# mit-acl/rl_collision_avoidance

Measured on AMD Instinct MI355X. Metric: agent-steps/sec (env.step) at 4 agents x 8192 worlds per GPU, higher is better.
Workload: dtype f64

## Files before the change

### include/cavoid.h

```cpp
#ifndef CAVOID_H
#define CAVOID_H
#include <stdint.h>

#ifdef __cplusplus
extern "C" {
#endif

#define CAVOID_ABI_VERSION 3
#define CAVOID_MAX_ACTIONS 32
#define CAVOID_MAX_AGENTS 64

#define CAVOID_F_AT_GOAL 0x01u
#define CAVOID_F_RAN_OUT 0x02u
#define CAVOID_F_IN_COLL 0x04u
#define CAVOID_F_WAS_AT_GOAL 0x08u
#define CAVOID_F_WAS_IN_COLL 0x10u
#define CAVOID_F_PRESENT 0x20u
#define CAVOID_F_LEARNING 0x40u
#define CAVOID_F_POLICY_SHIFT 8
#define CAVOID_F_POLICY_MASK 7u
enum { CAVOID_POLICY_EXTERNAL = 0, CAVOID_POLICY_STATIC = 1, CAVOID_POLICY_NONCOOP = 2, CAVOID_POLICY_RVO = 3, CAVOID_POLICY_FROZEN_NET = 4 };
#define CAVOID_F_DONE_MASK 0x07u

enum { CAVOID_SORT_CLOSEST_LAST = 0, CAVOID_SORT_CLOSEST_FIRST = 1, CAVOID_SORT_TIME_TO_IMPACT = 2 };
// ... 91 lines not shown
int cavoid_step_autoreset_n(cavoid_env *env, const int32_t *actions, int64_t action_stride, int32_t n_steps, int64_t out_step_stride,
                            float *obs, float *rewards, uint8_t *done, uint8_t *game_over, void *stream);

enum {
    CAVOID_FORM_NONE = 0,
    CAVOID_FORM_STEP = 1,
    CAVOID_FORM_QUAD = 2,
    CAVOID_FORM_RVO = 3,
    CAVOID_FORM_LOOP_PF = 4,
    CAVOID_FORM_LOOP = 5,
    CAVOID_FORM_PIPE = 6,
    CAVOID_FORM_RELAY = 7,
    CAVOID_FORM_CROWD = 8
};
int32_t cavoid_last_step_form(const cavoid_env *env, int32_t *relay_consumers);

int cavoid_step_continuous_autoreset(cavoid_env *env, const float *actions , float *obs, float *rewards, uint8_t *done,
                                     uint8_t *game_over, void *stream);
int cavoid_step_continuous_autoreset_n(cavoid_env *env, const float *actions, int64_t action_stride, int32_t n_steps, int64_t out_step_stride,
                                       float *obs, float *rewards, uint8_t *done, uint8_t *game_over, void *stream);

int32_t cavoid_packed_width(const cavoid_env *env);
int cavoid_reset_packed(cavoid_env *env, const uint8_t *world_mask, float *packed, void *stream);
int cavoid_observe_packed(cavoid_env *env, float *packed, void *stream);
int cavoid_step_packed(cavoid_env *env, const int32_t *actions, float *packed, uint8_t *game_over, void *stream);
int cavoid_step_autoreset_packed(cavoid_env *env, const int32_t *actions, int64_t action_stride, int32_t n_steps, int64_t out_step_stride,
                                 float *packed, uint8_t *game_over, void *stream);
int cavoid_step_continuous_autoreset_packed(cavoid_env *env, const float *actions, int64_t action_stride, int32_t n_steps,
                                            int64_t out_step_stride, float *packed, uint8_t *game_over, void *stream);

// ... 124 lines not shown
```

### rl_collision_avoidance_amd/_lib.py

```python
from __future__ import annotations

import ctypes as C
import os

from .build import LIB_PATH as _DEFAULT_LIB_PATH

LIB_PATH = os.environ.get("CAVOID_LIB", _DEFAULT_LIB_PATH)

MAX_ACTIONS = 32
MAX_AGENTS = 64
TILE_MAX_AGENTS = 16
ABI_VERSION = 3

F_AT_GOAL, F_RAN_OUT, F_IN_COLL, F_WAS_AT_GOAL, F_WAS_IN_COLL, F_PRESENT, F_LEARNING = 1, 2, 4, 8, 16, 32, 64
F_POLICY_SHIFT = 8
F_POLICY_MASK = 7
POLICY_EXTERNAL, POLICY_STATIC, POLICY_NONCOOP, POLICY_RVO, POLICY_FROZEN_NET = 0, 1, 2, 3, 4
F_DONE_MASK = 7
COMM_FORCE_RCCL = 1
STEP_FORMS = ("NONE", "STEP", "QUAD", "RVO", "LOOP_PF", "LOOP", "PIPE", "RELAY", "CROWD")


class CavoidCfg(C.Structure):
    _fields_ = [
# ... 53 lines not shown
        self.code = code


_P = C.c_void_p
SYMBOLS = [
    ("cavoid_abi_version", C.c_int, []),
    ("cavoid_strerror", C.c_char_p, [C.c_int]),
    ("cavoid_last_hip_error", C.c_int, []),
    ("cavoid_default_cfg", C.c_int, [C.POINTER(CavoidCfg), C.c_int32, C.c_int32]),
    ("cavoid_default_actions", C.c_int, [_P, C.POINTER(C.c_int32)]),
    ("cavoid_create", C.c_int, [C.POINTER(CavoidCfg), C.c_int64, C.c_int64, C.c_int, C.POINTER(_P)]),
    ("cavoid_destroy", None, [_P]),
    ("cavoid_num_worlds", C.c_int64, [_P]),
    ("cavoid_obs_width", C.c_int32, [_P]),
    ("cavoid_last_step_form", C.c_int32, [_P, C.POINTER(C.c_int32)]),
    ("cavoid_seed", C.c_int, [_P, C.c_uint64, _P, _P]),
    ("cavoid_get_episode", C.c_int, [_P, _P, _P]),
    ("cavoid_pool_refresh", C.c_int, [_P, C.c_uint32, _P]),
    ("cavoid_set_state", C.c_int, [_P, _P, _P, _P, _P]),
    ("cavoid_get_state", C.c_int, [_P, _P, _P, _P, _P]),
    ("cavoid_reset", C.c_int, [_P, _P, _P, _P]),
    ("cavoid_observe", C.c_int, [_P, _P, _P]),
    ("cavoid_step", C.c_int, [_P, _P, _P, _P, _P, _P, _P]),
    ("cavoid_step_continuous", C.c_int, [_P, _P, _P, _P, _P, _P, _P]),
    ("cavoid_step_autoreset", C.c_int, [_P, _P, _P, _P, _P, _P, _P]),
    ("cavoid_step_autoreset_n", C.c_int, [_P, _P, C.c_int64, C.c_int32, C.c_int64, _P, _P, _P, _P, _P]),
    ("cavoid_step_continuous_autoreset", C.c_int, [_P, _P, _P, _P, _P, _P, _P]),
    ("cavoid_step_continuous_autoreset_n", C.c_int, [_P, _P, C.c_int64, C.c_int32, C.c_int64, _P, _P, _P, _P, _P]),
    ("cavoid_step_continuous_autoreset_packed", C.c_int, [_P, _P, C.c_int64, C.c_int32, C.c_int64, _P, _P, _P]),
    ("cavoid_step_autoreset_n_timed", C.c_int, [_P, _P, C.c_int64, C.c_int32, C.c_int32, C.c_int64, _P, _P, _P, _P, _P, C.POINTER(C.c_float)]),
# ... 73 lines not shown
```

### rl_collision_avoidance_amd/batched_env.py

```python
from __future__ import annotations

import ctypes as C
from typing import Optional, Tuple

import numpy as np
import torch

from . import _lib
from .config import EnvConfig

_SORT = {"closest_last": 0, "closest_first": 1, "time_to_impact": 2}
_DYN = {"unicycle": 0, "unicycle_max_turn_rate": 1, "holonomic": 2}


def make_cfg(config: Optional[EnvConfig] = None, **overrides) -> _lib.CavoidCfg:
    config = config or EnvConfig()
    cfg = _lib.CavoidCfg()
    N = int(config.MAX_NUM_AGENTS_IN_ENVIRONMENT)
    M = int(config.MAX_NUM_OTHER_AGENTS_OBSERVED)
    _lib.check(_lib.lib().cavoid_default_cfg(C.byref(cfg), N, M), "cavoid_default_cfg")
    cfg.dt = config.DT
    cfg.near_goal_threshold = config.NEAR_GOAL_THRESHOLD
    cfg.max_time_ratio = config.MAX_TIME_RATIO
    cfg.collision_dist = config.COLLISION_DIST
# ... 181 lines not shown
    def refresh_pool(self, epoch: int) -> None:
        _lib.check(self._lib.cavoid_pool_refresh(self._h, int(epoch) & 0xFFFFFFFF, self._stream()), "cavoid_pool_refresh")

    @property
    def episode(self) -> torch.Tensor:
        out = torch.empty((self.num_worlds,), dtype=torch.int32, device=self.device)
        _lib.check(self._lib.cavoid_get_episode(self._h, self._ptr(out), self._stream()), "cavoid_get_episode")
        return out

    @property
    def last_step_form(self) -> Tuple[str, int]:
        nc = C.c_int32(0)
        form = self._lib.cavoid_last_step_form(self._h, C.byref(nc))
        return _lib.STEP_FORMS[form], int(nc.value)

    def set_state(self, state_f64: torch.Tensor, state_f32: torch.Tensor, flags: torch.Tensor) -> None:
        A = self.num_worlds * self.max_agents
        f64 = self._want(state_f64, (4, A), torch.float64, "state_f64")
        f32 = self._want(state_f32, (5, A), torch.float32, "state_f32")
        fl = self._want(flags, (A,), torch.int32, "flags")
        _lib.check(self._lib.cavoid_set_state(self._h, self._ptr(f64), self._ptr(f32), self._ptr(fl), self._stream()),
                   "cavoid_set_state")

    def get_state(self) -> Tuple[torch.Tensor, torch.Tensor, torch.Tensor]:
        A = self.num_worlds * self.max_agents
        f64 = torch.empty((4, A), dtype=torch.float64, device=self.device)
        f32 = torch.empty((5, A), dtype=torch.float32, device=self.device)
        fl = torch.empty((A,), dtype=torch.int32, device=self.device)
        _lib.check(self._lib.cavoid_get_state(self._h, self._ptr(f64), self._ptr(f32), self._ptr(fl), self._stream()),
                   "cavoid_get_state")
# ... 164 lines not shown
```

### rl_collision_avoidance_amd/csrc/cavoid_capi.hip

```cpp
#include <hip/hip_runtime.h>
#include <hip/hip_ext.h>

#include <cmath>
#include <cstdlib>
#include <cstring>
#include <new>

#include "cavoid.h"
#include "cavoid_host.hpp"
#include "cavoid_kernels.hpp"
#include "cavoid_launch.hpp"
#include "cavoid_crowd.hpp"

using namespace cavoid;

thread_local int g_last_hip_error = 0;

extern "C" int cavoid_abi_version(void) { return CAVOID_ABI_VERSION; }

extern "C" int cavoid_last_hip_error(void) { return g_last_hip_error; }

extern "C" const char *cavoid_strerror(int code) {
    switch (code) {
        case CAVOID_OK: return "ok";
// ... 333 lines not shown
    if (capturing) e->ahead_always = true;
    if (!e->ahead_always && e->ahead_primed && e->ahead_budget >= n_steps + 1) return CAVOID_OK;
    const int64_t waves = (e->W + e->k.wpw - 1) / e->k.wpw;
    const bool in_place = e->ahead_always;
    const dim3 grid((unsigned)((waves + 3) / 4), in_place ? 1u : (e->ahead_primed ? 4u : 32u)), block(256);
    const uint32_t *hi_in = e->ahead_hi[e->ahead_cur];
    uint32_t *hi_out = e->ahead_hi[in_place ? e->ahead_cur : (e->ahead_cur ^ 1)];
    hipEvent_t ev_fill = (timed_start && !capturing) ? *timed_start : nullptr;
    if (ev_fill) *timed_start = nullptr;
    const int rc = dispatch_n(e->cfg.max_agents, EnvNs{}, [&](auto n) -> int {
        launch_kernel(ahead_fill_kernel<decltype(n)::value>, grid, block, 0, s, ev_fill, nullptr, e->k, e->st.episode, hi_in, hi_out, e->pool, e->ahead_R);
        return CAVOID_OK;
    });
    if (rc != CAVOID_OK) return rc;
    HIP_TRY(hipGetLastError());
    if (!in_place) e->ahead_cur ^= 1;
    if (!capturing) { e->ahead_primed = true; e->ahead_budget = e->ahead_R; }
    return CAVOID_OK;
}
void cavoid_ahead_consumed(cavoid_env *e, int32_t n_steps) {
    if (!e || e->ahead_R <= 0) return;
    e->ahead_budget = e->ahead_budget > n_steps ? e->ahead_budget - n_steps : 0;
}

static int fill_pool(cavoid_env *e, hipStream_t s) {
    if (e->ahead_R > 0) {
        e->ahead_budget = 0;
        e->ahead_primed = false;
        HIP_TRY(hipMemsetAsync(e->ahead_hi[0], 0xFF, 2 * (size_t)e->W * sizeof(uint32_t), s));
        return CAVOID_OK;
    }
    if (e->pool_size <= 0) return CAVOID_OK;
    HIP_TRY(hipMemsetAsync(e->pool_episode, 0xFF, (size_t)e->pool_size * sizeof(uint32_t), s));
    KCfg k = e->k;
    k.num_worlds = e->pool_size;
    k.world_offset = 0;
    k.pool_size = 0;
    KState st{};
// ... 118 lines not shown
    return launch<MODE_STEP>(e, io, static_cast<hipStream_t>(stream));
}

static int launch_autoreset(cavoid_env *e, KIO io, const int32_t *actions, int64_t action_stride, int32_t n_steps, int64_t out_step_stride,
                            hipStream_t s, hipEvent_t ev_start = nullptr, hipEvent_t ev_stop = nullptr, const float *cont = nullptr) {
    if (e->cfg.dynamics == CAVOID_DYN_HOLONOMIC && !cont) return CAVOID_EINVAL;
    if (n_steps < 1 || action_stride < 0) return CAVOID_EINVAL;
    if (cont && n_steps > 1 && action_stride != 0 && action_stride < 2 * e->A) return CAVOID_EINVAL;
    if (out_step_stride != 0 && out_step_stride < e->W) return CAVOID_EINVAL;
    io.out_step_stride = n_steps > 1 ? out_step_stride : 0;
    io.actions = actions;
    io.cont = cont;
    io.action_stride = action_stride;
    io.n_steps = n_steps;
    e->last_form = CAVOID_FORM_NONE;
    if (int rc = cavoid_ahead_prepare(e, n_steps, s, &ev_start)) return rc;
    const int rc = (n_steps > 1 || e->prefetch_single)
                       ? cavoid_launch_multistep(e, io, e->latency_mode != 0, s, ev_start, ev_stop)
                       : launch<MODE_STEP_AUTORESET>(e, io, s, ev_start, ev_stop);
    cavoid_ahead_consumed(e, n_steps);
    return rc;
}

extern "C" int cavoid_step_autoreset(cavoid_env *e, const int32_t *actions, float *obs, float *rew, uint8_t *done, uint8_t *game_over, void *stream) {
    if (step_args(e, actions, rew, done, game_over) != CAVOID_OK) return CAVOID_EINVAL;
    return launch_autoreset(e, plain_io(e, obs, rew, done, game_over), actions, 0, 1, 0, static_cast<hipStream_t>(stream));
}

extern "C" int cavoid_step_autoreset_n(cavoid_env *e, const int32_t *actions, int64_t action_stride, int32_t n_steps, int64_t out_step_stride,
                                       float *obs, float *rew, uint8_t *done, uint8_t *game_over, void *stream) {
    if (step_args(e, actions, rew, done, game_over) != CAVOID_OK || n_steps < 0) return CAVOID_EINVAL;
    if (n_steps == 0) return CAVOID_OK;
    return launch_autoreset(e, plain_io(e, obs, rew, done, game_over), actions, action_stride, n_steps, out_step_stride,
                            static_cast<hipStream_t>(stream));
}
// ... 118 lines not shown
```

### rl_collision_avoidance_amd/csrc/cavoid_kernels.hpp

```cpp
#pragma once
#include <hip/hip_runtime.h>
#include <stdint.h>

#include "cavoid.h"

namespace cavoid {

#ifdef CAVOID_TRACE
__device__ unsigned long long *g_trace = nullptr;
#define CAVOID_STAMP(k)                                                                \
    do {                                                                               \
        if (lane == 0 && g_trace) g_trace[wave * 16 + (k)] = (unsigned long long)clock64(); \
    } while (0)
#else
#define CAVOID_STAMP(k) do { } while (0)
#endif

#define CAVOID_RARE(x) __builtin_expect(!!(x), 0)
#ifndef CAVOID_SKIP
#define CAVOID_SKIP 0
#endif

constexpr double kPi = 3.14159265358979323846;
constexpr int kTileMaxAgents = 16;
// ... 767 lines not shown
    a.gx = r.gx; a.gy = r.gy; a.radius = r.radius; a.pref = r.pref;
    a.flags = r.flags;
    a.vx = a.vy = 0.0;
    a.speed = 0.0f;
}

template <int N>
__device__ __forceinline__ void new_episode(const KCfg &c, const PoolRec *pool, uint32_t gw, uint32_t ep, int i, Agent &a) {
    if (c.pool_size > 0) {
        load_pool(pool, (int64_t)pool_index(c, gw, ep) * N + i, a);
    } else {
        generate_agent<N>(c, gw, ep, i, a);
    }
}

template <int N>
__device__ __forceinline__ void ahead_fill_wave(const KCfg &c, const uint32_t *episode, const uint32_t *hi_in, uint32_t *hi_out, PoolRec *ahead, const int need,
                                                const int64_t wave, const int lane, const int y, const int ny, double *sc_d, float *sc_r) {
    const int wpw = c.wpw, lanes_used = wpw * N;
    const int lw = lane / N, i = lane - lw * N;
    const int64_t w = wave * wpw + lw;
    const bool active = lane < lanes_used && w < c.num_worlds;
    const int base = lane < lanes_used ? lw * N : 0;
    uint32_t ep = 0u, fh = 0u;
    if (active) {
        ep = episode[w];
        fh = hi_in[w];
        if (fh == 0xFFFFFFFFu || (int32_t)(fh - ep) < 0) fh = ep;
    }
    const uint32_t target = ep + (uint32_t)need;
    int missing = active ? (int)(int32_t)(target - fh) : 0;
    missing = missing < 0 ? 0 : missing;
    int trips = missing;
#pragma unroll
    for (int o = 32; o > 0; o >>= 1) { const int v = __shfl_xor(trips, o, 64); trips = v > trips ? v : trips; }
    const uint32_t gw = (uint32_t)(c.world_offset + w);
    for (int k = y; k < trips; k += ny) {
        const uint32_t e = fh + 1u + (uint32_t)k;
        const bool fresh = active && k < missing;
        Agent a;
        absent_agent(a);
        if (c.gen_mode == 1) generate_world_v2<N>(c, gw, e, i, base, lane, fresh, sc_d, sc_d + 64, sc_d + 128, sc_d + 192, sc_r, a);
        else if (fresh) generate_agent<N>(c, gw, e, i, a);
        if (fresh) {
            PoolRec r;
            r.px = a.px; r.py = a.py; r.heading = a.heading; r.t_rem = a.t_rem;
            r.gx = a.gx; r.gy = a.gy; r.radius = a.radius; r.pref = a.pref;
            r.flags = a.flags; r.pad[0] = r.pad[1] = r.pad[2] = 0u;
            ahead[((int64_t)w * c.ahead + (int64_t)(e & (uint32_t)(c.ahead - 1))) * N + i] = r;
        }
    }
    if (active && i == 0 && y == 0) hi_out[w] = missing > 0 ? target : fh;
}

template <int N>
__global__ void __launch_bounds__(256) ahead_fill_kernel(const KCfg c, const uint32_t *episode, const uint32_t *hi_in, uint32_t *hi_out, PoolRec *ahead, const int need) {
    __shared__ double sh_d[4][4 * 64];
    __shared__ float sh_r[4][64];
    const int wave_in_block = threadIdx.x >> 6;
    ahead_fill_wave<N>(c, episode, hi_in, hi_out, ahead, need, (int64_t)blockIdx.x * 4 + wave_in_block, threadIdx.x & 63, (int)blockIdx.y, (int)gridDim.y,
                       sh_d[wave_in_block], sh_r[wave_in_block]);
}

constexpr double kRvoEps = 1e-5;
__device__ __forceinline__ double det2(double ax, double ay, double bx, double by) { return ax * by - ay * bx; }

struct Line { double px, py, dx, dy; };
// ... 731 lines not shown
```

### rl_collision_avoidance_amd/csrc/cavoid_launch.hpp

```cpp
#pragma once
#include <hip/hip_runtime.h>
#include <hip/hip_ext.h>

#include <type_traits>

#include "cavoid.h"
#include "cavoid_host.hpp"
#include "cavoid_kernels.hpp"

struct cavoid_env {
    int device = 0;
    int64_t W = 0, A = 0, world_offset = 0;
    cavoid_cfg cfg{};
    cavoid::KCfg k{};
    cavoid::KState st{};
    cavoid::PoolRec *pool = nullptr;
    uint32_t *pool_episode = nullptr;
    int64_t pool_size = 0;
    int ahead_R = 0;
    uint32_t *ahead_hi[2] = {nullptr, nullptr};
    int ahead_cur = 0;
    int ahead_budget = 0;
    bool ahead_primed = false;
    bool ahead_always = false;
    void *slab = nullptr;
    void *pool_slab = nullptr;
    double *d_actions = nullptr;
    int waves_per_block = 4;
    int grid = 0;
    int pipeline = 2;
    int relay_consumers = 3;
    int latency_mode = 0;
    int quad = -1;
    int prefetch_single = 0;
    int last_form = CAVOID_FORM_NONE;
    int last_relay_consumers = 0;
    hipEvent_t ev0 = nullptr, ev1 = nullptr;
};

// ... 28 lines not shown

template <class K, class... Args>
static inline void launch_kernel(K kernel, dim3 grid, dim3 block, size_t lds, hipStream_t s, hipEvent_t ev_start, hipEvent_t ev_stop,
                                 const Args &...args) {
    if (ev_start || ev_stop) hipExtLaunchKernelGGL(kernel, grid, block, lds, s, ev_start, ev_stop, 0, args...);
    else hipLaunchKernelGGL(kernel, grid, block, lds, s, args...);
}

#ifdef CAVOID_TRACE
static inline int set_trace(unsigned long long *dev_ptr) {
    HIP_TRY(hipMemcpyToSymbol(HIP_SYMBOL(g_trace), &dev_ptr, sizeof(dev_ptr)));
    return CAVOID_OK;
}
#endif

static inline int note_form(cavoid_env *e, int rc, int form, int relay_consumers = 0) {
    if (rc == CAVOID_OK) {
        e->last_form = form;
        e->last_relay_consumers = relay_consumers;
    }
    return rc;
}

template <int MODE, bool RVO = false>
static inline int launch_on(cavoid_env *e, const KCfg &k, const KState &st, int grid_x, const KIO &io, hipStream_t s,
                     hipEvent_t ev_start, hipEvent_t ev_stop) {
    const dim3 grid(grid_x), block(64 * e->waves_per_block);
    const int row = io.obs ? io.obs_stride : k.width;
    int tile = (k.tile_rows * row + 3) & ~3;
    if (tile < k.park_floats) tile = k.park_floats;
// ... 24 lines not shown
        constexpr int N = decltype(n)::value;
        const size_t lds = pipe_lds_fixed_bytes<N>() + tail;
        if (lds > 65536) return CAVOID_EUNSUPPORTED;
        launch_kernel(env_pipe_kernel<N, RVO>, grid, block, lds, s, ev_start, ev_stop, k, e->st, e->pool, io);
        return CAVOID_OK;
    });
    if (rc != CAVOID_OK) return rc;
    HIP_TRY(hipGetLastError());
    return CAVOID_OK;
}

}

int cavoid_ahead_prepare(cavoid_env *e, int32_t n_steps, hipStream_t s, hipEvent_t *timed_start = nullptr);
void cavoid_ahead_consumed(cavoid_env *e, int32_t n_steps);
int cavoid_launch_relay(cavoid_env *e, const cavoid::KIO &io, hipStream_t s, hipEvent_t ev_start, hipEvent_t ev_stop);
int cavoid_launch_quad(cavoid_env *e, const cavoid::KIO &io, hipStream_t s, hipEvent_t ev_start, hipEvent_t ev_stop);
int cavoid_launch_multistep(cavoid_env *e, const cavoid::KIO &io, bool prefetch, hipStream_t s, hipEvent_t ev_start, hipEvent_t ev_stop);
int cavoid_launch_rvo(cavoid_env *e, int mode, const cavoid::KIO &io, hipStream_t s, hipEvent_t ev_start, hipEvent_t ev_stop);
int cavoid_launch_crowd(cavoid_env *e, int mode, const cavoid::KCfg &k, const cavoid::KState &st, int64_t worlds, const cavoid::KIO &io,
                        hipStream_t s, hipEvent_t ev_start, hipEvent_t ev_stop);
#ifdef CAVOID_TRACE
int cavoid_debug_trace_multistep(unsigned long long *dev_ptr);
int cavoid_debug_trace_rvo(unsigned long long *dev_ptr);
int cavoid_debug_trace_relay(unsigned long long *dev_ptr);
int cavoid_debug_trace_quad(unsigned long long *dev_ptr);
#endif
```

### rl_collision_avoidance_amd/csrc/cavoid_relay.hip

```cpp
#include "cavoid_launch.hpp"
#include "cavoid_relay.hpp"

using namespace cavoid;

template <int N>
static int relay_allow_lds() {
    static bool allowed = false;
    if (!allowed) {
        HIP_TRY(hipFuncSetAttribute(reinterpret_cast<const void *>(env_relay_kernel<N>), hipFuncAttributeMaxDynamicSharedMemorySize, (int)kRelayLdsLimit));
        allowed = true;
    }
    return CAVOID_OK;
}

int cavoid_launch_relay(cavoid_env *e, const KIO &io, hipStream_t s, hipEvent_t ev_start, hipEvent_t ev_stop) {
    const KCfg &k = e->k;
    if (k.rvo_enabled || k.pool_size <= 0 || !io.obs || !io.actions || io.cont) return CAVOID_EUNSUPPORTED;
    if (k.switches & kSwSkipDonePairs) return CAVOID_EUNSUPPORTED;
    const int64_t tiles = (e->W + k.wpw - 1) / k.wpw;
    if (tiles > 512) return CAVOID_EUNSUPPORTED;
    if (e->cfg.max_agents > kRelayMaxAgents) return CAVOID_EUNSUPPORTED;
    const int row = io.obs_stride;
    const int tile_floats = (k.tile_rows * row + 3) & ~3;
    if (k.tile_rows < k.wpw * e->cfg.max_agents) return CAVOID_EUNSUPPORTED;
    const dim3 grid((unsigned)tiles);
    int used_nc = 0;
    const int rc = dispatch_n(e->cfg.max_agents, RelayNs{}, [&](auto n) -> int {
        constexpr int N = decltype(n)::value;
        int nc = e->relay_consumers;
        while (nc > 1 && relay_lds_fixed_bytes<N>() + (size_t)nc * tile_floats * sizeof(float) > kRelayLdsLimit) --nc;
        const size_t lds = relay_lds_fixed_bytes<N>() + (size_t)nc * tile_floats * sizeof(float);
        if (lds > kRelayLdsLimit || (nc < 2 && e->relay_consumers >= 2)) return CAVOID_EUNSUPPORTED;
        if (lds > 65536) {
            const int rc_opt = relay_allow_lds<N>();
            if (rc_opt != CAVOID_OK) return rc_opt;
        }
        used_nc = nc;
        launch_kernel(env_relay_kernel<N>, grid, dim3(64 * (3 + nc)), lds, s, ev_start, ev_stop, k, e->st, e->pool, io);
        return CAVOID_OK;
    });
    if (rc != CAVOID_OK) return rc;
    HIP_TRY(hipGetLastError());
    return note_form(e, CAVOID_OK, CAVOID_FORM_RELAY, used_nc);
}

#ifdef CAVOID_TRACE
int cavoid_debug_trace_relay(unsigned long long *dev_ptr) { return set_trace(dev_ptr); }
#endif
```

### rl_collision_avoidance_amd/csrc/cavoid_relay.hpp

```cpp
#pragma once
#include "cavoid_kernels.hpp"

namespace cavoid {

constexpr int kRelayMaxAgents = 6;
template <int N>
__host__ __device__ constexpr int relay_ring() { return N <= 5 ? 8 : 4; }
constexpr size_t kRelayLdsLimit = 80 * 1024;
constexpr int kRelayActRing = 64;
constexpr int kRelayActAhead = 48;
constexpr int kRelayEvq = 8;

struct RelaySeq {
    int spec;
    int stage;
    int res;
    int fin;
    int act;
    int ev;
    int nxt;
    int cons[kRelayMaxConsumers];
    int cfin[kRelayMaxConsumers];
    int coop[2];
    int kernarg[2];
// ... 8 lines not shown
#endif
#ifndef CAVOID_RELAY_PRIO_D
#define CAVOID_RELAY_PRIO_D 3
#endif
#ifndef CAVOID_RELAY_PRIO_P
#define CAVOID_RELAY_PRIO_P 3
#endif
#ifndef CAVOID_RELAY_PRIO_L
#define CAVOID_RELAY_PRIO_L 0
#endif
#ifndef CAVOID_RELAY_PRIO_C
#define CAVOID_RELAY_PRIO_C 1
#endif
#ifndef CAVOID_RELAY_ABL
#define CAVOID_RELAY_ABL 0
#endif
__device__ __forceinline__ int relay_role_of(int wv, int NC) {
    if (NC == 3) return (int)(((unsigned)CAVOID_RELAY_ORDER >> (4 * wv)) & 15u);
    return wv;
}
constexpr int kRelayCoopWaves = 3;
constexpr int kRelayCoopFromN = 4;
template <int N>
struct RelayCoop {
    static constexpr int K = Others<N>::K;
    uint64_t key[K][64];
    uint32_t bits[K][64];
};
template <int N>
__host__ __device__ constexpr size_t relay_coop_bytes() { return N >= kRelayCoopFromN ? sizeof(RelayCoop<N>) : 0; }
// ... 204 lines not shown
        neighbour_features(e, (float)e.prll_x, (float)e.prll_y, rx, ry, q, feat[o]);
    }
}

struct RelayArgs { KCfg c; KState s; const PoolRec *pool; KIO io; };
template <class T>
__device__ __forceinline__ void relay_load_args(T &dst, const __attribute__((address_space(4))) T *src) {
    static_assert(sizeof(T) % 4 == 0, "whole words");
    const __attribute__((address_space(4))) uint32_t *w = (const __attribute__((address_space(4))) uint32_t *)src;
    uint32_t d[sizeof(T) / 4];
#pragma unroll
    for (int k = 0; k < (int)(sizeof(T) / 4); ++k) d[k] = w[k];
    __builtin_memcpy(&dst, d, sizeof(T));
}
template <int N>
__device__ __forceinline__ void relay_coop_last(unsigned char *smem) {
    unsigned char *sp = smem + lds_floats_block() * sizeof(float);
    RelaySeq *seq = reinterpret_cast<RelaySeq *>(sp); sp += sizeof(RelaySeq) + kRelayEvq * sizeof(unsigned long long);
    const unsigned long long kp = (unsigned long long)(uint32_t)relay_peek(&seq->kernarg[0]) | ((unsigned long long)(uint32_t)relay_peek(&seq->kernarg[1]) << 32);
    typedef const __attribute__((address_space(4))) RelayArgs *ArgP;
    const ArgP ka = (ArgP)kp;
    KCfg c;
    KIO io;
    relay_load_args(c, &ka->c);
    relay_load_args(io, &ka->io);
    RelayTent *tents = reinterpret_cast<RelayTent *>(sp); sp += relay_ring<N>() * sizeof(RelayTent) + sizeof(RelayNxt);
    RelayRes *ress = reinterpret_cast<RelayRes *>(sp); sp += relay_ring<N>() * sizeof(RelayRes) + kRelayActRing * 64;
    RelayCoop<N> *coopb = reinterpret_cast<RelayCoop<N> *>(sp); sp += relay_coop_bytes<N>();
    float *tiles = reinterpret_cast<float *>(sp);
    const int lane0 = threadIdx.x & 63;
// ... 39 lines not shown
        gapf[o] = 0.0f;
#pragma unroll
        for (int q = 0; q < kFeat; ++q) feat[o][q] = 0.0f;
    }
    if (c.switches != 0u) relay_pair_part<N, true>(c, ao, e, present, as, pw, lane0, co, gapf, feat);
    else relay_pair_part<N, false>(c, ao, e, present, as, pw, lane0, co, gapf, feat);
    relay_coop_arrive(&seq->coop[0], lane0);
    Key key[K];
    uint32_t valid = 0u;
    if (N == 1) key[0].set(kKeySentinel, 0u);
#pragma unroll
    for (int o = 0; o < N - 1; ++o) {
        key[o].v = co.key[o][lane0];
        valid |= (co.bits[o][lane0] & 2u) ? (1u << o) : 0u;
    }
    if (t - NC >= 0) relay_wait_bounded(&seq->cons[cid_l], t - NC + 1);
    const int rows_active = (int)worlds_here * N;
    assemble_obs<N, false, true, ArrayStage<N>, NoHook, false, PartOthers>(c, ao, e, active, lane0, as, key, gapf, feat, valid, tile, nullptr,
                                                                           rows_active, ostride, false, 0.0f, 0.0f, wave, NoHook(), false, nullptr,
                                                                           PartOthers{pw, kRelayCoopWaves});
    if (pw == 0 && active && lane0 < rows_active) {
        const int M = c.max_other;
        const int m = __popc(valid);
        const int first = m > M ? m - M : 0;
        const int kept = m - first;
        write_row_head(tile + lane0 * ostride, ao, e, present, kept, kept, M, packed, c.width, rew_c, done_c);
    }
    relay_coop_arrive(&seq->coop[1], lane0);
    if (io.out_step_stride == 0)
        for (int o = 0; o < NC; ++o) relay_wait_bounded(&seq->cfin[o], 1);
// ... 3 lines not shown
        const bool lines = ((rows_active * ostride) & 31) == 0 && (reinterpret_cast<uintptr_t>(dst) & 127) == 0;
        if (io.out_step_stride != 0 && lines) flush_tile<4, true, true>(tile, dst, rows_active * ostride, pw * 64 + lane0, 64 * kRelayCoopWaves);
        else if (io.out_step_stride != 0) flush_tile<4, true>(tile, dst, rows_active * ostride, pw * 64 + lane0, 64 * kRelayCoopWaves);
        else flush_tile<4>(tile, dst, rows_active * ostride, pw * 64 + lane0, 64 * kRelayCoopWaves);
    }
    if (pw == 0 && active) {
        if (!packed) {
            io.rew[slot_w * N + a_idx0] = rew_c;
            io.done[slot_w * N + a_idx0] = (ctl_c & 1u) ? 1 : 0;
        }
        if (i0 == 0) io.game_over[slot_w + w] = (ctl_c & 2u) ? 1 : 0;
    }
    if (pw == 0) RELAY_MARK(29);
}

template <int N>
__global__ void __launch_bounds__(64 * (3 + kRelayMaxConsumers), 1) env_relay_kernel(const KCfg c, const KState s, const PoolRec *pool, const KIO io) {
    extern __shared__ __attribute__((aligned(16))) unsigned char smem[];
    unsigned char *sp = smem;
    double *lds_tab = reinterpret_cast<double *>(sp); sp += lds_floats_block() * sizeof(float);
    RelaySeq *seq = reinterpret_cast<RelaySeq *>(sp); sp += sizeof(RelaySeq);
    unsigned long long *evq = reinterpret_cast<unsigned long long *>(sp); sp += kRelayEvq * sizeof(unsigned long long);
    RelayTent *tents = reinterpret_cast<RelayTent *>(sp); sp += relay_ring<N>() * sizeof(RelayTent);
    RelayNxt *nbuf = reinterpret_cast<RelayNxt *>(sp); sp += sizeof(RelayNxt);
    RelayRes *ress = reinterpret_cast<RelayRes *>(sp); sp += relay_ring<N>() * sizeof(RelayRes);
    unsigned char *actring = sp; sp += kRelayActRing * 64;
    RelayCoop<N> *coopb = reinterpret_cast<RelayCoop<N> *>(sp); sp += relay_coop_bytes<N>();
    float *tiles = reinterpret_cast<float *>(sp);

    const int NC = (blockDim.x >> 6) - 3;
    const int role = relay_role_of(threadIdx.x >> 6, NC);
    const int lane0 = threadIdx.x & 63;
// ... 4 lines not shown
    const int64_t w0 = wave * wpw;
    const int lw = lane0 / N, i0 = lane0 - lw * N;
    const int64_t w = w0 + lw;
    const bool active = lane0 < lanes_used && w < c.num_worlds;
    const int base0 = lane0 < lanes_used ? lw * N : 0;
    const int64_t a_idx0 = w * N + i0;
    const bool packed = io.packed != 0;
    int64_t worlds_here = c.num_worlds - w0;
    if (worlds_here > wpw) worlds_here = wpw;
    if (worlds_here < 0) worlds_here = 0;
    const int n_steps = io.n_steps;
    constexpr bool kCoop = N >= kRelayCoopFromN;
    const bool coop_role = role < 2 || role == 2 + NC;

    if (role == 0 && lane0 < (int)(sizeof(RelaySeq) / sizeof(int))) reinterpret_cast<int *>(seq)[lane0] = 0;
    if constexpr (kCoop) {
        if (role == 0 && lane0 == 0) {
            const unsigned long long kp = (unsigned long long)__builtin_amdgcn_kernarg_segment_ptr();
            seq->kernarg[0] = (int)(uint32_t)kp; seq->kernarg[1] = (int)(uint32_t)(kp >> 32);
            seq->tile_id = (int)blockIdx.x;
        }
    }

    if (role == 0) {
        __builtin_amdgcn_s_setprio(CAVOID_RELAY_PRIO_D);
        RELAY_MARK(20);
        KCfg cd = c;
        asm volatile("" : "+s"(cd.dt), "+s"(cd.near_goal_sq), "+s"(cd.actions_fp32), "+s"(cd.dynamics),
                     "+s"(cd.timeout_enabled), "+s"(cd.switches));
        const RelayTrig trig = relay_trig_constants();
        Agent a;
        a.px = a.py = a.heading = a.t_rem = a.vx = a.vy = 0.0;
        a.gx = a.gy = a.radius = a.pref = a.speed = 0.0f;
        a.flags = 0u;
        uint32_t episode = 0u;
        double tab_v = 0.0;
        if (lane0 < 2 * c.num_actions) tab_v = c.action_table[lane0];
        int act0 = 0;
        if (active) {
            episode = s.episode[w];
            load_agent(s, a_idx0, a);
            act0 = io.actions[a_idx0];
        }
        if (cd.actions_fp32 && (lane0 & 1)) tab_v = (double)(float)tab_v;
        lds_tab[lane0] = tab_v;
        act0 = act0 < 0 ? 0 : (act0 >= c.num_actions ? c.num_actions - 1 : act0);
        const bool present_first = active && (a.flags & CAVOID_F_PRESENT);
        bool restarted_any = false, moved_any = false;
        int events = 0;
        bool T_moving;
        Agent T;
        wave_lds_sync();
        RelayStatics ks = relay_statics(a, active);
        T = relay_advance(cd, trig, a, ks, lds_tab[2 * act0], lds_tab[2 * act0 + 1], active, T_moving);
        __syncthreads();
// ... 105 lines not shown
            S.flags = vflags;
            const bool restart = (ctl & 2u) != 0u;
            if (__ballot(restart) != 0ull) {
                relay_wait(&seq->nxt, events + 1);
                Agent nx;
                relay_read_nxt(*nbuf, lane0, nx);
                if (restart) {
                    S = nx; episode += 1u; restarted_any = true;
                    stage_out(tents[t & (relay_ring<N>() - 1)], nx, relay_statics(nx, active).r_staged, lane0);
                    res->flags[lane0] = nx.flags;
                }
            }
            relay_post(&seq->fin, t + 1);
        }
        RELAY_MARK(23);
        relay_post(&seq->stage, n_steps + 1);
        if (restarted_any) {
            store_agent(s, a_idx0, S);
            if (i0 == 0) s.episode[w] = episode;
        } else if (present_first) {
            if (moved_any) {
                s.px[a_idx0] = S.px; s.py[a_idx0] = S.py; s.heading[a_idx0] = S.heading; s.t_rem[a_idx0] = S.t_rem;
            }
            s.speed[a_idx0] = S.speed;
            s.flags[a_idx0] = S.flags;
        }
        RELAY_MARK(24);
    } else if (role == 1) {
        __builtin_amdgcn_s_setprio(CAVOID_RELAY_PRIO_P);
        KCfg cp = c;
// ... 126 lines not shown
                relay_post(&seq->act, loaded);
                continue;
            }
            if (fin >= n_steps && relay_peek(&seq->stage) > n_steps) break;
            if (++idle_polls > kRelayPollLimit) __builtin_trap();
            __builtin_amdgcn_s_sleep(2);
        }
    } else {
        __builtin_amdgcn_s_setprio(CAVOID_RELAY_PRIO_C);
        KCfg cc = c;
        asm volatile("" : "+s"(cc.switches));
        const int cid = role - 2;
        float *tile = tiles + (size_t)cid * tile_floats;
        __syncthreads();
        const int n_mine = kCoop ? n_steps - 1 : n_steps;
        for (int t = cid; t < n_mine; t += NC) {
            int lane = lane0, i = i0, base = base0;
            asm volatile("" : "+v"(lane), "+v"(i), "+v"(base));
            RELAY_STAMP(16);
            relay_wait_bounded(&seq->fin, t + 1);
            RELAY_STAMP(17);
            if (CAVOID_RELAY_ABL & 1) { relay_post(&seq->cons[cid], t + 1); continue; }
            const RelayTent &f = tents[t & (relay_ring<N>() - 1)];
            const RelayRes &v = ress[t & (relay_ring<N>() - 1)];
            Agent ao;
            ao.px = f.px[lane]; ao.py = f.py[lane]; ao.vx = f.vx[lane]; ao.vy = f.vy[lane];
            ao.heading = f.heading[lane]; ao.t_rem = 0.0;
            ao.gx = f.gx[lane]; ao.gy = f.gy[lane]; ao.speed = 0.0f;
            ao.radius = f.r[lane]; ao.pref = f.pref[lane]; ao.flags = v.flags[lane];
            const uint32_t ctl_c = v.ctl[lane];
            const float rew_c = v.rew[lane], done_c = (ctl_c & 1u) ? 1.0f : 0.0f;
// ... 21 lines not shown
            if (active) {
                if (!packed) {
                    io.rew[slot_w * N + a_idx0] = rew_c;
                    io.done[slot_w * N + a_idx0] = (ctl_c & 1u) ? 1 : 0;
                }
                if (i0 == 0) io.game_over[slot_w + w] = (ctl_c & 2u) ? 1 : 0;
            }
            relay_post(&seq->cons[cid], t + 1);
            RELAY_STAMP(19);
            if (t == 0) RELAY_MARK(28);
            if (t == n_steps - 1) RELAY_MARK(29);
        }
        __builtin_amdgcn_s_waitcnt(0);
        if (cid == 0) RELAY_MARK(30);
        relay_post(&seq->cfin[cid], 1);
    }
    if constexpr (kCoop) {
        if (coop_role) relay_coop_last<N>(smem);
    }
}

}
```

Baseline: 23.67 billion.

## Refill ahead-generated episode pool inside relay kernel tail instead of separate launch

```diff
diff --git a/include/cavoid.h b/include/cavoid.h
--- a/include/cavoid.h
+++ b/include/cavoid.h
@@ -129,6 +129,7 @@
     CAVOID_FORM_CROWD = 8
 };
 int32_t cavoid_last_step_form(const cavoid_env *env, int32_t *relay_consumers);
+int64_t cavoid_ahead_refill_launches(const cavoid_env *env);
 
 int cavoid_step_continuous_autoreset(cavoid_env *env, const float *actions , float *obs, float *rewards, uint8_t *done,
                                      uint8_t *game_over, void *stream);
diff --git a/rl_collision_avoidance_amd/_lib.py b/rl_collision_avoidance_amd/_lib.py
--- a/rl_collision_avoidance_amd/_lib.py
+++ b/rl_collision_avoidance_amd/_lib.py
@@ -91,6 +91,7 @@
     ("cavoid_num_worlds", C.c_int64, [_P]),
     ("cavoid_obs_width", C.c_int32, [_P]),
     ("cavoid_last_step_form", C.c_int32, [_P, C.POINTER(C.c_int32)]),
+    ("cavoid_ahead_refill_launches", C.c_int64, [_P]),
     ("cavoid_seed", C.c_int, [_P, C.c_uint64, _P, _P]),
     ("cavoid_get_episode", C.c_int, [_P, _P, _P]),
     ("cavoid_pool_refresh", C.c_int, [_P, C.c_uint32, _P]),
diff --git a/rl_collision_avoidance_amd/batched_env.py b/rl_collision_avoidance_amd/batched_env.py
--- a/rl_collision_avoidance_amd/batched_env.py
+++ b/rl_collision_avoidance_amd/batched_env.py
@@ -219,6 +219,10 @@
         form = self._lib.cavoid_last_step_form(self._h, C.byref(nc))
         return _lib.STEP_FORMS[form], int(nc.value)
 
+    @property
+    def ahead_refill_launches(self) -> int:
+        return int(self._lib.cavoid_ahead_refill_launches(self._h))
+
     def set_state(self, state_f64: torch.Tensor, state_f32: torch.Tensor, flags: torch.Tensor) -> None:
         A = self.num_worlds * self.max_agents
         f64 = self._want(state_f64, (4, A), torch.float64, "state_f64")
diff --git a/rl_collision_avoidance_amd/csrc/cavoid_capi.hip b/rl_collision_avoidance_amd/csrc/cavoid_capi.hip
--- a/rl_collision_avoidance_amd/csrc/cavoid_capi.hip
+++ b/rl_collision_avoidance_amd/csrc/cavoid_capi.hip
@@ -371,6 +371,7 @@
     });
     if (rc != CAVOID_OK) return rc;
     HIP_TRY(hipGetLastError());
+    e->ahead_refill_launches += 1;
     if (!in_place) e->ahead_cur ^= 1;
     if (!capturing) { e->ahead_primed = true; e->ahead_budget = e->ahead_R; }
     return CAVOID_OK;
@@ -379,6 +380,19 @@
     if (!e || e->ahead_R <= 0) return;
     e->ahead_budget = e->ahead_budget > n_steps ? e->ahead_budget - n_steps : 0;
 }
+
+void cavoid_ahead_launched(cavoid_env *e, int32_t n_steps, int rc) {
+    if (!e || e->ahead_R <= 0) return;
+    const bool filled = e->ahead_tail_filled;
+    e->ahead_tail_filled = false;
+    if (rc == CAVOID_OK && filled && e->last_form == CAVOID_FORM_RELAY && relay_refills_rings(e)) {
+        e->ahead_cur ^= 1;
+        e->ahead_budget = e->ahead_R;
+        return;
+    }
+    cavoid_ahead_consumed(e, n_steps);
+}
+extern "C" int64_t cavoid_ahead_refill_launches(const cavoid_env *e) { return e ? e->ahead_refill_launches : 0; }
 
 static int fill_pool(cavoid_env *e, hipStream_t s) {
     if (e->ahead_R > 0) {
@@ -527,11 +541,12 @@
     io.action_stride = action_stride;
     io.n_steps = n_steps;
     e->last_form = CAVOID_FORM_NONE;
+    e->ahead_tail_filled = false;
     if (int rc = cavoid_ahead_prepare(e, n_steps, s, &ev_start)) return rc;
     const int rc = (n_steps > 1 || e->prefetch_single)
                        ? cavoid_launch_multistep(e, io, e->latency_mode != 0, s, ev_start, ev_stop)
                        : launch<MODE_STEP_AUTORESET>(e, io, s, ev_start, ev_stop);
-    cavoid_ahead_consumed(e, n_steps);
+    cavoid_ahead_launched(e, n_steps, rc);
     return rc;
 }
 
diff --git a/rl_collision_avoidance_amd/csrc/cavoid_kernels.hpp b/rl_collision_avoidance_amd/csrc/cavoid_kernels.hpp
--- a/rl_collision_avoidance_amd/csrc/cavoid_kernels.hpp
+++ b/rl_collision_avoidance_amd/csrc/cavoid_kernels.hpp
@@ -805,9 +805,9 @@
     }
 }
 
-template <int N>
-__device__ __forceinline__ void ahead_fill_wave(const KCfg &c, const uint32_t *episode, const uint32_t *hi_in, uint32_t *hi_out, PoolRec *ahead, const int need,
-                                                const int64_t wave, const int lane, const int y, const int ny, double *sc_d, float *sc_r) {
+template <int N, bool V2, class Load>
+__device__ __forceinline__ void ahead_fill_lanes(const KCfg &c, Load load, uint32_t *hi_out, PoolRec *ahead, const int need,
+                                                 const int64_t wave, const int lane, const int y, const int ny, double *sc_d, float *sc_r) {
     const int wpw = c.wpw, lanes_used = wpw * N;
     const int lw = lane / N, i = lane - lw * N;
     const int64_t w = wave * wpw + lw;
@@ -815,8 +815,7 @@
     const int base = lane < lanes_used ? lw * N : 0;
     uint32_t ep = 0u, fh = 0u;
     if (active) {
-        ep = episode[w];
-        fh = hi_in[w];
+        load(w, ep, fh);
         if (fh == 0xFFFFFFFFu || (int32_t)(fh - ep) < 0) fh = ep;
     }
     const uint32_t target = ep + (uint32_t)need;
@@ -830,8 +829,8 @@
         const uint32_t e = fh + 1u + (uint32_t)k;
         const bool fresh = active && k < missing;
         Agent a;
-        absent_agent(a);
-        if (c.gen_mode == 1) generate_world_v2<N>(c, gw, e, i, base, lane, fresh, sc_d, sc_d + 64, sc_d + 128, sc_d + 192, sc_r, a);
+        if (V2) absent_agent(a);
+        if (V2 && c.gen_mode == 1) generate_world_v2<N>(c, gw, e, i, base, lane, fresh, sc_d, sc_d + 64, sc_d + 128, sc_d + 192, sc_r, a);
         else if (fresh) generate_agent<N>(c, gw, e, i, a);
         if (fresh) {
             PoolRec r;
@@ -842,6 +841,12 @@
         }
     }
     if (active && i == 0 && y == 0) hi_out[w] = missing > 0 ? target : fh;
+}
+template <int N>
+__device__ __forceinline__ void ahead_fill_wave(const KCfg &c, const uint32_t *episode, const uint32_t *hi_in, uint32_t *hi_out, PoolRec *ahead, const int need,
+                                                const int64_t wave, const int lane, const int y, const int ny, double *sc_d, float *sc_r) {
+    ahead_fill_lanes<N, true>(c, [&](int64_t w, uint32_t &ep, uint32_t &fh) { ep = episode[w]; fh = hi_in[w]; }, hi_out, ahead, need, wave, lane, y, ny,
+                              sc_d, sc_r);
 }
 
 template <int N>
diff --git a/rl_collision_avoidance_amd/csrc/cavoid_launch.hpp b/rl_collision_avoidance_amd/csrc/cavoid_launch.hpp
--- a/rl_collision_avoidance_amd/csrc/cavoid_launch.hpp
+++ b/rl_collision_avoidance_amd/csrc/cavoid_launch.hpp
@@ -23,6 +23,8 @@
     int ahead_budget = 0;
     bool ahead_primed = false;
     bool ahead_always = false;
+    bool ahead_tail_filled = false;
+    int64_t ahead_refill_launches = 0;
     void *slab = nullptr;
     void *pool_slab = nullptr;
     double *d_actions = nullptr;
@@ -81,6 +83,17 @@
 }
 #endif
 
+constexpr int kRelayFillFromN = 2, kRelayFillToN = 4;
+static inline bool relay_refills_rings(const cavoid_env *e) {
+#ifdef CAVOID_DEV_NO_TAIL_REFILL
+    (void)e;
+    return false;
+#else
+    return e->ahead_R > 0 && e->k.gen_mode == 0 && !e->ahead_always && e->cfg.max_agents >= kRelayFillFromN &&
+           e->cfg.max_agents <= kRelayFillToN;
+#endif
+}
+
 static inline int note_form(cavoid_env *e, int rc, int form, int relay_consumers = 0) {
     if (rc == CAVOID_OK) {
         e->last_form = form;
@@ -135,6 +148,7 @@
 
 int cavoid_ahead_prepare(cavoid_env *e, int32_t n_steps, hipStream_t s, hipEvent_t *timed_start = nullptr);
 void cavoid_ahead_consumed(cavoid_env *e, int32_t n_steps);
+void cavoid_ahead_launched(cavoid_env *e, int32_t n_steps, int rc);
 int cavoid_launch_relay(cavoid_env *e, const cavoid::KIO &io, hipStream_t s, hipEvent_t ev_start, hipEvent_t ev_stop);
 int cavoid_launch_quad(cavoid_env *e, const cavoid::KIO &io, hipStream_t s, hipEvent_t ev_start, hipEvent_t ev_stop);
 int cavoid_launch_multistep(cavoid_env *e, const cavoid::KIO &io, bool prefetch, hipStream_t s, hipEvent_t ev_start, hipEvent_t ev_stop);
diff --git a/rl_collision_avoidance_amd/csrc/cavoid_relay.hip b/rl_collision_avoidance_amd/csrc/cavoid_relay.hip
--- a/rl_collision_avoidance_amd/csrc/cavoid_relay.hip
+++ b/rl_collision_avoidance_amd/csrc/cavoid_relay.hip
@@ -8,6 +8,9 @@
     static bool allowed = false;
     if (!allowed) {
         HIP_TRY(hipFuncSetAttribute(reinterpret_cast<const void *>(env_relay_kernel<N>), hipFuncAttributeMaxDynamicSharedMemorySize, (int)kRelayLdsLimit));
+        if constexpr (N >= kRelayFillFromN && N <= kRelayFillToN)
+            HIP_TRY(hipFuncSetAttribute(reinterpret_cast<const void *>(env_relay_kernel<N, RelayFillPtrs>), hipFuncAttributeMaxDynamicSharedMemorySize,
+                                        (int)kRelayLdsLimit));
         allowed = true;
     }
     return CAVOID_OK;
@@ -24,6 +27,7 @@
     const int tile_floats = (k.tile_rows * row + 3) & ~3;
     if (k.tile_rows < k.wpw * e->cfg.max_agents) return CAVOID_EUNSUPPORTED;
     const dim3 grid((unsigned)tiles);
+    const bool fill = relay_refills_rings(e);
     int used_nc = 0;
     const int rc = dispatch_n(e->cfg.max_agents, RelayNs{}, [&](auto n) -> int {
         constexpr int N = decltype(n)::value;
@@ -36,11 +40,17 @@
             if (rc_opt != CAVOID_OK) return rc_opt;
         }
         used_nc = nc;
-        launch_kernel(env_relay_kernel<N>, grid, dim3(64 * (3 + nc)), lds, s, ev_start, ev_stop, k, e->st, e->pool, io);
+        if constexpr (N >= kRelayFillFromN && N <= kRelayFillToN) {
+            if (fill)
+                launch_kernel(env_relay_kernel<N, RelayFillPtrs>, grid, dim3(64 * (3 + nc)), lds, s, ev_start, ev_stop, k, e->st, e->pool, io,
+                              RelayFillPtrs{e->ahead_hi[e->ahead_cur], e->ahead_hi[e->ahead_cur ^ 1]});
+        }
+        if (!fill) launch_kernel(env_relay_kernel<N>, grid, dim3(64 * (3 + nc)), lds, s, ev_start, ev_stop, k, e->st, e->pool, io);
         return CAVOID_OK;
     });
     if (rc != CAVOID_OK) return rc;
     HIP_TRY(hipGetLastError());
+    e->ahead_tail_filled = fill;
     return note_form(e, CAVOID_OK, CAVOID_FORM_RELAY, used_nc);
 }
 
diff --git a/rl_collision_avoidance_amd/csrc/cavoid_relay.hpp b/rl_collision_avoidance_amd/csrc/cavoid_relay.hpp
--- a/rl_collision_avoidance_amd/csrc/cavoid_relay.hpp
+++ b/rl_collision_avoidance_amd/csrc/cavoid_relay.hpp
@@ -46,6 +46,9 @@
 #endif
 #ifndef CAVOID_RELAY_ABL
 #define CAVOID_RELAY_ABL 0
+#endif
+#ifndef CAVOID_RELAY_TAIL_FORM
+#define CAVOID_RELAY_TAIL_FORM 1
 #endif
 __device__ __forceinline__ int relay_role_of(int wv, int NC) {
     if (NC == 3) return (int)(((unsigned)CAVOID_RELAY_ORDER >> (4 * wv)) & 15u);
@@ -280,6 +283,8 @@
     __builtin_memcpy(&dst, d, sizeof(T));
 }
 template <int N>
+__device__ __forceinline__ void relay_tail_refill(unsigned char *smem, const int y, const int ny);
+template <int N, bool FILL>
 __device__ __forceinline__ void relay_coop_last(unsigned char *smem) {
     unsigned char *sp = smem + lds_floats_block() * sizeof(float);
     RelaySeq *seq = reinterpret_cast<RelaySeq *>(sp); sp += sizeof(RelaySeq) + kRelayEvq * sizeof(unsigned long long);
@@ -349,6 +354,7 @@
         key[o].v = co.key[o][lane0];
         valid |= (co.bits[o][lane0] & 2u) ? (1u << o) : 0u;
     }
+    if constexpr (FILL && CAVOID_RELAY_TAIL_FORM == 1) relay_tail_refill<N>(smem, pw == 1 ? 0 : (pw == 0 ? 1 : 2), kRelayCoopWaves);
     if (t - NC >= 0) relay_wait_bounded(&seq->cons[cid_l], t - NC + 1);
     const int rows_active = (int)worlds_here * N;
     assemble_obs<N, false, true, ArrayStage<N>, NoHook, false, PartOthers>(c, ao, e, active, lane0, as, key, gapf, feat, valid, tile, nullptr,
@@ -382,8 +388,40 @@
     if (pw == 0) RELAY_MARK(29);
 }
 
+struct RelayFillPtrs { const uint32_t *hi_in; uint32_t *hi_out; };
+struct RelayFillArgs { RelayArgs a; RelayFillPtrs p; };
+static_assert(sizeof(RelayArgs) % alignof(RelayFillPtrs) == 0, "the fifth argument follows the fourth without padding");
+static_assert(2 * 64 * sizeof(uint32_t) <= lds_floats_block() * sizeof(float), "D's hand-over fits the action table's words");
+__device__ __forceinline__ const uint32_t *relay_fill_hi_in() { return nullptr; }
+__device__ __forceinline__ const uint32_t *relay_fill_hi_in(const RelayFillPtrs &p) { return p.hi_in; }
 template <int N>
-__global__ void __launch_bounds__(64 * (3 + kRelayMaxConsumers), 1) env_relay_kernel(const KCfg c, const KState s, const PoolRec *pool, const KIO io) {
+__device__ __forceinline__ void relay_tail_refill(unsigned char *smem, const int y, const int ny) {
+    unsigned char *sp = smem + lds_floats_block() * sizeof(float);
+    RelaySeq *seq = reinterpret_cast<RelaySeq *>(sp);
+    const unsigned long long kp = (unsigned long long)(uint32_t)relay_peek(&seq->kernarg[0]) | ((unsigned long long)(uint32_t)relay_peek(&seq->kernarg[1]) << 32);
+    typedef const __attribute__((address_space(4))) RelayFillArgs *ArgP;
+    const ArgP ka = (ArgP)kp;
+    KCfg c;
+    relay_load_args(c, &ka->a.c);
+    KCold cold;
+    relay_load_args(cold, (const __attribute__((address_space(4))) KCold *)(unsigned long long)c.cold);
+    c.cold = &cold;
+    const int n_steps = ka->a.io.n_steps;
+    const int lane0 = threadIdx.x & 63;
+    const int64_t wave = relay_peek(&seq->tile_id);
+    relay_wait_bounded(&seq->stage, n_steps + 1);
+    const uint32_t ep_mine = reinterpret_cast<const uint32_t *>(smem)[lane0], fh_mine = reinterpret_cast<const uint32_t *>(smem)[64 + lane0];
+    if (y == 0) RELAY_MARK(14);
+    ahead_fill_lanes<N, false>(c, [&](int64_t, uint32_t &ep, uint32_t &fh) { ep = ep_mine; fh = fh_mine; }, ka->p.hi_out, const_cast<PoolRec *>(ka->a.pool),
+                               c.ahead, wave, lane0, y, ny, nullptr, nullptr);
+    if (y == 0) RELAY_MARK(15);
+}
+
+template <int N, class... Fill>
+__global__ void __launch_bounds__(64 * (3 + kRelayMaxConsumers), 1) env_relay_kernel(const KCfg c, const KState s, const PoolRec *pool, const KIO io,
+                                                                                      const Fill... fill_ptrs) {
+    static_assert(sizeof...(Fill) <= 1, "at most the one RelayFillPtrs");
+    constexpr bool FILL = sizeof...(Fill) != 0;
     extern __shared__ __attribute__((aligned(16))) unsigned char smem[];
     unsigned char *sp = smem;
     double *lds_tab = reinterpret_cast<double *>(sp); sp += lds_floats_block() * sizeof(float);
@@ -418,7 +456,7 @@
     const bool coop_role = role < 2 || role == 2 + NC;
 
     if (role == 0 && lane0 < (int)(sizeof(RelaySeq) / sizeof(int))) reinterpret_cast<int *>(seq)[lane0] = 0;
-    if constexpr (kCoop) {
+    if constexpr (kCoop || FILL) {
         if (role == 0 && lane0 == 0) {
             const unsigned long long kp = (unsigned long long)__builtin_amdgcn_kernarg_segment_ptr();
             seq->kernarg[0] = (int)(uint32_t)kp; seq->kernarg[1] = (int)(uint32_t)(kp >> 32);
@@ -438,11 +476,13 @@
         a.gx = a.gy = a.radius = a.pref = a.speed = 0.0f;
         a.flags = 0u;
         uint32_t episode = 0u;
+        uint32_t filled_hi = 0u;
         double tab_v = 0.0;
         if (lane0 < 2 * c.num_actions) tab_v = c.action_table[lane0];
         int act0 = 0;
         if (active) {
             episode = s.episode[w];
+            if constexpr (FILL) filled_hi = relay_fill_hi_in(fill_ptrs...)[w];
             load_agent(s, a_idx0, a);
             act0 = io.actions[a_idx0];
         }
@@ -578,6 +618,10 @@
             relay_post(&seq->fin, t + 1);
         }
         RELAY_MARK(23);
+        if constexpr (FILL) {
+            reinterpret_cast<uint32_t *>(lds_tab)[lane0] = episode;
+            reinterpret_cast<uint32_t *>(lds_tab)[64 + lane0] = filled_hi;
+        }
         relay_post(&seq->stage, n_steps + 1);
         if (restarted_any) {
             store_agent(s, a_idx0, S);
@@ -734,7 +778,8 @@
         float *tile = tiles + (size_t)cid * tile_floats;
         __syncthreads();
         const int n_mine = kCoop ? n_steps - 1 : n_steps;
-        for (int t = cid; t < n_mine; t += NC) {
+        int t = cid;
+        for (; t < n_mine; t += NC) {
             int lane = lane0, i = i0, base = base0;
             asm volatile("" : "+v"(lane), "+v"(i), "+v"(base));
             RELAY_STAMP(16);
@@ -786,10 +831,11 @@
         __builtin_amdgcn_s_waitcnt(0);
         if (cid == 0) RELAY_MARK(30);
         relay_post(&seq->cfin[cid], 1);
+        if constexpr (FILL && !(kCoop && CAVOID_RELAY_TAIL_FORM == 1)) relay_tail_refill<N>(smem, t - n_mine, NC);
     }
     if constexpr (kCoop) {
-        if (coop_role) relay_coop_last<N>(smem);
-    }
-}
-
-}
+        if (coop_role) relay_coop_last<N, FILL>(smem);
+    }
+}
+
+}
```

After: 23.95 billion, median of 6. 1.2% higher.
